# zyhbili/Dual-Space-NeRF

Measured on AMD Instinct MI355X. Metric: rendered rays/sec (64 samples/ray), 512x512 frame, higher is better.
Workload: dtype split-f16x3 (3 x v_mfma_f32_32x32x16_f16 on hi/lo fp16 operand halves, f32 accumulate: f32-equivalent accuracy - parity bars of the tests: 1e-4 absolute on RGB / acc / weights against the reference; sigma 1e-4 absolute where |sigma| <= 100 and 4e-6 RELATIVE to max|sigma| above (this checkpoint: |sig

## Files before the change

dual-space-nerf_amd/csrc/dsn_field16.hip:

```cpp
#include "dsn_common.h"
#include "dsn_kernels.h"

typedef float f32x16 __attribute__((ext_vector_type(16)));
typedef _Float16 half8 __attribute__((ext_vector_type(8)));
#define MFMA16(a, b, c) __builtin_amdgcn_mfma_f32_32x32x16_f16((a), (b), (c), 0, 0, 0)

#if !defined(DSN_EXPERIMENTS) && (defined(F16_ABL) || defined(F16_SABL) || defined(F16_TIMING) || defined(F16_TRAIN_ABL))
#error "F16_ABL / F16_SABL / F16_TIMING are experiment switches (wrong results / debug counters): build with -DDSN_EXPERIMENTS"
#endif
#ifndef F16_SINCOS_OCML
#define F16_SINCOS_OCML 0
#endif
#ifndef F16_FENCE
#define F16_FENCE 0
#endif
#ifndef F16_SGB
#define F16_SGB 1
#endif
#ifndef F16_SGB_VALU
#define F16_SGB_VALU 2
#endif
#ifndef F16_SGB_DS
#define F16_SGB_DS 1
#endif
#ifndef F16_MIX
#define F16_MIX 1
#endif
#ifndef F16_PIPE_LATE
#define F16_PIPE_LATE 1
#endif
#ifndef F16_ABL
#define F16_ABL 0
#endif
#ifndef F16_NEXT_POINT
#define F16_NEXT_POINT 1
#endif
#ifndef F16_DMA_SPREAD
#define F16_DMA_SPREAD 1
#endif
#ifndef F16_BIAS_AHEAD
#define F16_BIAS_AHEAD 1
#endif
#ifndef F16_TIMING
#define F16_TIMING 0
#endif
#ifndef F16_PREFETCH
#define F16_PREFETCH 1
#endif

#define F16_THREADS 256
#if defined(DSN_EXPERIMENTS) && defined(F16_TRAIN_ABL) && (F16_TRAIN_ABL & 32)
#define F16_ST_M(m) (1024 * (m))
#else
#define F16_ST_M(m) (32 * (m))
#endif
#define F16_CHUNK 8
#define F16_RING_SLOTS (2 * F16_CHUNK)
#define F16_NCHUNK (DSN_STREAM_BLOCKS / F16_CHUNK)
#define F16_RANGE 65000.0f
#define F16_RANGE_SCALED 32768.0f
#define F16_GSCALE 0.015625f
#define F16_GUNSCALE 64.0f

#if F16_TIMING
__device__ unsigned long long g_f16_timing[16];
#define F16_STAMP(i) do { if (MODE == F16_FWD) { asm volatile("s_waitcnt vmcnt(0) lgkmcnt(0)" ::: "memory"); tstamp[i] = __builtin_readcyclecounter(); rstamp[i] = wall_clock64(); } } while (0)
extern "C" __attribute__((visibility("default"))) int dsn_debug_timing(unsigned long long* out16, int reset) {
    if (out16 && hipMemcpyFromSymbol(out16, HIP_SYMBOL(g_f16_timing), sizeof(unsigned long long) * 16) != hipSuccess) return 1;
    if (reset) { unsigned long long z[16] = {0}; if (hipMemcpyToSymbol(HIP_SYMBOL(g_f16_timing), z, sizeof(z)) != hipSuccess) return 1; }
    return 0;
}
#else
#define F16_STAMP(i) do { } while (0)
#endif
struct W16 {
    const char* g;
    char* ring;
    unsigned ring_off;
    int wave;
    int nchunk = F16_NCHUNK;
    bool spread = F16_DMA_SPREAD != 0;
    half8 h0, l0, h1, l1;
};

#ifndef F16_POS_OFFS
#define F16_POS_OFFS 0
#endif
__device__ __forceinline__ void w16_stage(const W16& w, int c) {
    const char* src = w.g + (size_t)c * 32768;
    const unsigned dst = w.ring_off + (c & 1) * 32768 + w.wave * 8192 + 4096;
#if F16_POS_OFFS
    asm volatile("s_mov_b32 m0, %1\n\ts_nop 0\n\t"
                 "global_load_lds_dwordx4 %0, off\n\tglobal_load_lds_dwordx4 %0, off offset:1024\n\t"
                 "global_load_lds_dwordx4 %0, off offset:2048\n\tglobal_load_lds_dwordx4 %0, off offset:3072"
                 : : "v"(src - 4096), "s"(dst - 4096) : "memory", "m0");
    asm volatile("s_mov_b32 m0, %1\n\ts_nop 0\n\t"
                 "global_load_lds_dwordx4 %0, off\n\tglobal_load_lds_dwordx4 %0, off offset:1024\n\t"
                 "global_load_lds_dwordx4 %0, off offset:2048\n\tglobal_load_lds_dwordx4 %0, off offset:3072"
                 : : "v"(src), "s"(dst) : "memory", "m0");
    return;
#endif
    asm volatile("s_mov_b32 m0, %1\n\ts_nop 0\n\t"
                 "global_load_lds_dwordx4 %0, off offset:-4096\n\tglobal_load_lds_dwordx4 %0, off offset:-3072\n\t"
                 "global_load_lds_dwordx4 %0, off offset:-2048\n\tglobal_load_lds_dwordx4 %0, off offset:-1024\n\t"
                 "global_load_lds_dwordx4 %0, off\n\tglobal_load_lds_dwordx4 %0, off offset:1024\n\t"
                 "global_load_lds_dwordx4 %0, off offset:2048\n\tglobal_load_lds_dwordx4 %0, off offset:3072"
                 : : "v"(src), "s"(dst) : "memory", "m0");
}
template <int I>
__device__ __forceinline__ void w16_stage_part(const W16& w, int c) {
    const char* src = w.g + (size_t)c * 32768;
    const unsigned dst = w.ring_off + (c & 1) * 32768 + w.wave * 8192 + 4096;
#if F16_POS_OFFS
    {
        const int back = I < 2 ? 4096 : 0;
        asm volatile("s_mov_b32 m0, %1\n\ts_nop 0\n\t"
                     "global_load_lds_dwordx4 %0, off offset:%2\n\tglobal_load_lds_dwordx4 %0, off offset:%3"
                     : : "v"(src - back), "s"(dst - back), "n"(2048 * (I & 1)), "n"(2048 * (I & 1) + 1024) : "memory", "m0");
        return;
    }
#endif
    asm volatile("s_mov_b32 m0, %1\n\ts_nop 0\n\t"
                 "global_load_lds_dwordx4 %0, off offset:%2\n\tglobal_load_lds_dwordx4 %0, off offset:%3"
                 : : "v"(src), "s"(dst), "n"(-4096 + 2048 * I), "n"(-3072 + 2048 * I) : "memory", "m0");
}
__device__ __forceinline__ void w16_boundary(const W16& w, int b) {
#if !(F16_ABL & 2)
    asm volatile("s_waitcnt vmcnt(0)" ::: "memory");
#endif
#if !(F16_ABL & 1)
    __syncthreads();
#endif
    const int c = b / F16_CHUNK;
#if !(F16_ABL & 4)
    if (!w.spread && c + 1 < w.nchunk) w16_stage(w, c + 1);
#endif
}
__device__ __forceinline__ void w16_read(const W16& w, int b, int lane, half8& h0, half8& l0, half8& h1, half8& l1) {
    const char* s = w.ring + ((b >> 3) & 1) * 32768 + (b & 7) * 1024 + lane * 16;
    h0 = *reinterpret_cast<const half8*>(s);
    l0 = *reinterpret_cast<const half8*>(s + 8192);
    h1 = *reinterpret_cast<const half8*>(s + 16384);
    l1 = *reinterpret_cast<const half8*>(s + 24576);
}
__device__ __forceinline__ void w16_begin_issue(W16& w, int first_blk) { w16_stage(w, first_blk / F16_CHUNK); }
__device__ __forceinline__ void w16_begin_wait(W16& w, int lane, int first_blk) {
    w16_boundary(w, first_blk);
#if !(F16_ABL & 4)
    if (w.spread && first_blk / F16_CHUNK + 1 < w.nchunk) w16_stage_part<0>(w, first_blk / F16_CHUNK + 1);
#endif
    w16_read(w, first_blk, lane, w.h0, w.l0, w.h1, w.l1);
}
__device__ __forceinline__ void w16_begin(W16& w, int lane, int first_blk) {
    w16_begin_issue(w, first_blk);
    w16_begin_wait(w, lane, first_blk);
}

struct NoHook { __device__ __forceinline__ void operator()(int) const {} };

template <int KB, bool XLS, class Hook = NoHook>
__device__ __forceinline__ void dense16(W16& w, int& blk, int lane, const half8 (&xh)[KB][2], const half8 (&xl)[KB][2],
                                        f32x16& accM, f32x16& accC, Hook&& hook = NoHook()) {
#pragma unroll
    for (int kb = 0; kb < KB; ++kb) {
#if F16_PREFETCH
        half8 n0 = w.h0, m0 = w.l0, n1 = w.h1, m1 = w.l1;
        if (blk + 1 < DSN_STREAM_BLOCKS) {
            if (((blk + 1) & (F16_CHUNK - 1)) == 0) w16_boundary(w, blk + 1);
#if !(F16_ABL & 4)
            if (w.spread) {
                const int pos = (blk + 1) & (F16_CHUNK - 1), cn = (blk + 1) / F16_CHUNK + 1;
                if (cn < w.nchunk) {
                    if (pos == 0) w16_stage_part<0>(w, cn);
                    if (pos == 1) w16_stage_part<1>(w, cn);
                    if (pos == 2) w16_stage_part<2>(w, cn);
                    if (pos == 3) w16_stage_part<3>(w, cn);
                }
            }
#endif
            w16_read(w, blk + 1, lane, n0, m0, n1, m1);
        }
#else
        if (blk > 0) {
            if ((blk & (F16_CHUNK - 1)) == 0) w16_boundary(w, blk);
            w16_read(w, blk, lane, w.h0, w.l0, w.h1, w.l1);
        }
#endif
        if (XLS) {
            accM = MFMA16(w.h0, xh[kb][0], accM);
            accC = MFMA16(w.h0, xl[kb][0], accC);
            accC = MFMA16(w.l0, xh[kb][0], accC);
            accM = MFMA16(w.h1, xh[kb][1], accM);
            accC = MFMA16(w.h1, xl[kb][1], accC);
            accC = MFMA16(w.l1, xh[kb][1], accC);
        } else {
            accM = MFMA16(w.h0, xh[kb][0], accM);
            accC = MFMA16(w.l0, xh[kb][0], accC);
            accM = MFMA16(w.h0, xl[kb][0], accM);
            accC = MFMA16(w.h1, xh[kb][1], accC);
            accM = MFMA16(w.l1, xh[kb][1], accM);
            accC = MFMA16(w.h1, xl[kb][1], accC);
        }
#if !(F16_ABL & 8)
        hook(kb);
#endif
#if F16_PREFETCH
        w.h0 = n0; w.l0 = m0; w.h1 = n1; w.l1 = m1;
#endif
        ++blk;
#if F16_SGB
#pragma unroll
        for (int i = 0; i < 6; ++i) {
            __builtin_amdgcn_sched_group_barrier(0x008, 1, 0);
#if F16_SGB_DS
            if (i < 4) __builtin_amdgcn_sched_group_barrier(0x100, 1, 0);
#endif
            __builtin_amdgcn_sched_group_barrier(0x002, F16_SGB_VALU, 0);
        }
        __builtin_amdgcn_sched_barrier(0);
#endif
#if F16_FENCE
        __builtin_amdgcn_sched_barrier(0);
#endif
    }
}

__device__ __forceinline__ f32x16 rows16(const float* __restrict__ v, int m, int half) {
    f32x16 o;
#pragma unroll
    for (int q = 0; q < 4; ++q) {
        const float4 t = *reinterpret_cast<const float4*>(v + 32 * m + 8 * q + 4 * half);
        o[4 * q + 0] = t.x; o[4 * q + 1] = t.y; o[4 * q + 2] = t.z; o[4 * q + 3] = t.w;
    }
    return o;
}
__device__ __forceinline__ f32x16 zero16() {
    f32x16 z;
#pragma unroll
    for (int r = 0; r < 16; ++r) z[r] = 0.0f;
    return z;
}
template <bool SCALED>
__device__ __forceinline__ void split16(const f32x16& v, half8 (&h)[2], half8 (&l)[2]) {
#pragma unroll
    for (int r = 0; r < 16; ++r) {
        const _Float16 hi = (_Float16)v[r];
        const float res = fmaf((float)hi, -1.0f, v[r]);
        h[r >> 3][r & 7] = hi;
        l[r >> 3][r & 7] = SCALED ? (_Float16)(res * DSN_LO_SCALE) : (_Float16)res;
    }
}
#define F16_FWD_SCALE 64.0f
#define F16_FWD_INV 0.015625f
__device__ __forceinline__ f32x16 unscale16(const f32x16& m, const f32x16& c) {
    f32x16 v;
#pragma unroll
    for (int r = 0; r < 16; ++r) v[r] = (m[r] + c[r]) * F16_FWD_INV;
    return v;
}
__device__ __forceinline__ f32x16 fold16(const f32x16& m, const f32x16& c) {
    f32x16 v;
#pragma unroll
    for (int r = 0; r < 16; ++r) v[r] = fmaf(c[r], DSN_LO_INV, m[r]);
    return v;
}
__device__ __forceinline__ uint32_t dsn_push_sign(uint32_t word, float v) {
    return __builtin_amdgcn_alignbit(word, __float_as_uint(v), 31);
}
__device__ __forceinline__ uint32_t dsn_active_word(uint32_t signs) { return ~signs & 0xffffu; }
#ifndef F16_KEEP_ASM
#define F16_KEEP_ASM 1
#endif
__device__ __forceinline__ float dsn_keep_active(float v, uint32_t word, int r) {
#if F16_KEEP_ASM
    uint32_t m;
    asm("v_bfe_i32 %0, %1, %2, 1" : "=v"(m) : "v"(word), "s"(15 - r));
    return __uint_as_float(__float_as_uint(v) & m);
#else
    return __uint_as_float(__float_as_uint(v) & (uint32_t)__builtin_amdgcn_sbfe((int)word, 15 - r, 1));
#endif
}
__device__ __forceinline__ uint32_t relu_bits16(f32x16& a) {
    uint32_t s = 0;
#pragma unroll
    for (int r = 0; r < 16; ++r) {
        s = dsn_push_sign(s, a[r]);
        a[r] = fmaxf(a[r], 0.0f);
    }
    return dsn_active_word(s);
}
__device__ __forceinline__ void mask16(f32x16& a, uint32_t m) {
#pragma unroll
    for (int r = 0; r < 16; ++r) a[r] = dsn_keep_active(a[r], m, r);
}

__device__ __forceinline__ void track16(float& ovf, const f32x16& v) {
#pragma unroll
    for (int r = 0; r < 16; r += 2) asm("v_max3_f32 %0, %0, |%1|, |%2|" : "+v"(ovf) : "v"(v[r]), "v"(v[r + 1]));
}
__device__ __forceinline__ float dsn_nan_flag() { return __uint_as_float(0x7fc00000u); }

#if defined(DSN_EXPERIMENTS) && defined(F16_TRAIN_ABL) && (F16_TRAIN_ABL & 256)
__device__ __forceinline__ void store16_lines_emul(float* st, const float (&o)[16]) {
    const int lane = threadIdx.x & 63;
    const unsigned long long me = (unsigned long long)(uintptr_t)st;
#pragma unroll
    for (int j = 0; j < 4; ++j) {
        const int src = 8 * j + (lane >> 3);
        const unsigned lo = __shfl((unsigned)me, src), hi = __shfl((unsigned)(me >> 32), src);
        float* pj = reinterpret_cast<float*>((uintptr_t)(((unsigned long long)hi << 32) | lo));
        if (pj) *reinterpret_cast<float4*>(pj + 4 * (lane & 7)) = make_float4(o[4 * j], o[4 * j + 1], o[4 * j + 2], o[4 * j + 3]);
    }
}
#endif
template <bool FWD, bool ST = false, bool HEAD = false>
__device__ __forceinline__ void epi_slice(const f32x16& pM, const f32x16& pC, int kb, uint32_t mword, uint32_t& bits,
                                          half8 (&yh)[2], half8 (&yl)[2], float& ovf, float* st = nullptr, float stscale = 1.0f,
                                          const float* wd = nullptr, float* sg = nullptr) {
#if F16_ABL & 16
    {
        asm volatile("" : : "a"(pM[2 * kb]), "a"(pM[2 * kb + 1]), "a"(pC[2 * kb]), "a"(pC[2 * kb + 1]));
        if (kb == 0) { yh[0] = yh[1]; yl[0] = yl[1]; }
        return;
    }
#endif
    float vv[2];
#pragma unroll
    for (int e = 0; e < 2; ++e) {
        const int r = 2 * kb + e;
// ... 71 lines not shown
    }
}
#ifndef F16_NT_STORE
#define F16_NT_STORE 0
#endif
typedef float f32x4 __attribute__((ext_vector_type(4)));
__device__ __forceinline__ void store16(float* st, const f32x16& v, float stscale) {
#if defined(DSN_EXPERIMENTS) && defined(F16_TRAIN_ABL) && (F16_TRAIN_ABL & 4)
    {
        const int lane = threadIdx.x & 63, hf = lane >> 5, i = lane & 3;
        const unsigned long long me = (unsigned long long)(uintptr_t)st;
#pragma unroll
        for (int j = 0; j < 4; ++j) {
            const int src = (lane & ~3) | j;
            const unsigned lo = __shfl((unsigned)me, src), hi = __shfl((unsigned)(me >> 32), src);
            float* pj = reinterpret_cast<float*>((uintptr_t)(((unsigned long long)hi << 32) | lo));
            if (pj) *reinterpret_cast<float4*>(pj - 4 * hf + 16 * hf + 4 * i) =
                make_float4(v[4 * j] * stscale, v[4 * j + 1] * stscale, v[4 * j + 2] * stscale, v[4 * j + 3] * stscale);
        }
        return;
    }
#endif
#if defined(DSN_EXPERIMENTS) && defined(F16_TRAIN_ABL) && (F16_TRAIN_ABL & 256)
    {
        float o[16];
#pragma unroll
        for (int r = 0; r < 16; ++r) o[r] = v[r] * stscale;
        store16_lines_emul(st, o);
        return;
    }
#endif
    if (!st) return;
#pragma unroll
    for (int q = 0; q < 4; ++q) {
#if F16_NT_STORE
        const f32x4 x = {v[4 * q] * stscale, v[4 * q + 1] * stscale, v[4 * q + 2] * stscale, v[4 * q + 3] * stscale};
        __builtin_nontemporal_store(x, reinterpret_cast<f32x4*>(st + 8 * q));
#else
        *reinterpret_cast<float4*>(st + 8 * q) = make_float4(v[4 * q] * stscale, v[4 * q + 1] * stscale, v[4 * q + 2] * stscale, v[4 * q + 3] * stscale);
#endif
    }
}

template <bool ST = false, bool EXTRA = false, bool HEAD = false>
__device__ __forceinline__ void layer16_fwd(W16& w, int& blk, int lane, const float* __restrict__ bias,
                                            const half8 (&xh)[8][2], const half8 (&xl)[8][2], half8 (&yh)[8][2],
                                            half8 (&yl)[8][2], uint32_t (&mk)[4], float& ovf, float* st = nullptr,
                                            const half8 (*s_pe)[F16_THREADS] = nullptr, const float* wden = nullptr, float* sg = nullptr) {
    const int half = lane >> 5;
    const int tid = threadIdx.x;
    f32x16 pM = zero16(), pC = zero16();
#if F16_BIAS_AHEAD
    f32x16 bnext = rows16(bias, 0, half);
#endif
#pragma unroll
    for (int m = 0; m < 8; ++m) {
#if F16_BIAS_AHEAD
        f32x16 aM = bnext, aC = zero16();
        if (m + 1 < 8) bnext = rows16(bias, m + 1, half);
#else
        f32x16 aM = rows16(bias, m, half), aC = zero16();
#endif
        uint32_t bits = 0;
        if (m == 0) dense16<8, false>(w, blk, lane, xh, xl, aM, aC);
        else dense16<8, false>(w, blk, lane, xh, xl, aM, aC, [&](int kb) {
            epi_slice<true, ST, HEAD>(pM, pC, kb, 0u, bits, yh[m - 1], yl[m - 1], ovf, (ST && st) ? st + F16_ST_M(m - 1) : nullptr, 1.0f,
                                      HEAD ? wden + 32 * (m - 1) + 4 * half : nullptr, sg); });
        if (EXTRA) {
            half8 qh[2][2], ql[2][2];
            qh[0][0] = s_pe[0][tid]; qh[0][1] = s_pe[1][tid]; qh[1][0] = s_pe[2][tid]; qh[1][1] = s_pe[3][tid];
            ql[0][0] = s_pe[4][tid]; ql[0][1] = s_pe[5][tid]; ql[1][0] = s_pe[6][tid]; ql[1][1] = s_pe[7][tid];
            dense16<2, false>(w, blk, lane, qh, ql, aM, aC);
        }
        if (m > 0) { if ((m - 1) & 1) mk[(m - 1) >> 1] |= dsn_active_word(bits) << 16; else mk[(m - 1) >> 1] = dsn_active_word(bits); }
        pM = aM; pC = aC;
    }
    {
        uint32_t bits = 0;
#pragma unroll
        for (int kb = 0; kb < 8; ++kb)
            epi_slice<true, ST, HEAD>(pM, pC, kb, 0u, bits, yh[7], yl[7], ovf, (ST && st) ? st + F16_ST_M(7) : nullptr, 1.0f,
                                      HEAD ? wden + 32 * 7 + 4 * half : nullptr, sg);
        mk[3] |= dsn_active_word(bits) << 16;
    }
}
template <bool ST = false>
__device__ __forceinline__ void layer16_bwd(W16& w, int& blk, int lane, const half8 (&xh)[8][2],
                                            const half8 (&xl)[8][2], half8 (&yh)[8][2], half8 (&yl)[8][2],
                                            const uint32_t (&mk)[4], float& ovf, float* st = nullptr, float stscale = F16_GUNSCALE) {
    f32x16 pM = zero16(), pC = zero16();
    uint32_t dummy = 0;
#pragma unroll
    for (int m = 0; m < 8; ++m) {
        f32x16 aM = zero16(), aC = zero16();
        const uint32_t mw = m > 0 ? ((mk[(m - 1) >> 1] >> (16 * ((m - 1) & 1))) & 0xffffu) : 0u;
        if (m == 0) dense16<8, true>(w, blk, lane, xh, xl, aM, aC);
        else dense16<8, true>(w, blk, lane, xh, xl, aM, aC, [&](int kb) { epi_slice<false, ST>(pM, pC, kb, mw, dummy, yh[m - 1], yl[m - 1], ovf, (ST && st) ? st + F16_ST_M(m - 1) : nullptr, stscale); });
        pM = aM; pC = aC;
    }
    const uint32_t mw = (mk[3] >> 16) & 0xffffu;
#pragma unroll
    for (int kb = 0; kb < 8; ++kb) epi_slice<false, ST>(pM, pC, kb, mw, dummy, yh[7], yl[7], ovf, (ST && st) ? st + F16_ST_M(7) : nullptr, stscale);
}

#define F16_FULL 0
#define F16_FWD 1
#define F16_BWD 2
#define F16_TRAIN 3
#define F16_DEN 4
#define F16_FIRST_BWD_BLOCK (OFF_L6T / DSN_BLK)
#define F16_DEN_BLOCKS (F16_FIRST_BWD_BLOCK - 4 * 8)
static_assert(F16_DEN_BLOCKS % F16_CHUNK == 0, "the density-only kernel streams whole chunks");
template <int MODE>
__global__ void __launch_bounds__(F16_THREADS, 1)
k_field16(const float* __restrict__ packed, const DsnFrameState* __restrict__ fs, const float* __restrict__ x_c,
          int64_t N, const int32_t* __restrict__ active_list, const int32_t* __restrict__ active_count,
          float* __restrict__ sigma, float* __restrict__ essence, float* __restrict__ grad,
          uint4* __restrict__ masks, int32_t* __restrict__ pos_list, int32_t* __restrict__ pos_count,
          float* __restrict__ tr_h, float* __restrict__ tr_a, float* __restrict__ tr_rr, int64_t slot_base, int64_t rec_cap,
          const int32_t* __restrict__ sel, int32_t* __restrict__ flag_count) {
    constexpr bool ST = MODE == F16_TRAIN;
    __shared__ __attribute__((aligned(16))) char ring[F16_RING_SLOTS * 4096];
    __shared__ uint32_t s_mask[7][4][F16_THREADS];
    __shared__ __attribute__((aligned(16))) float s_vec[256 + 2304 + 8];
    __shared__ __attribute__((aligned(16))) half8 s_pe[8][F16_THREADS];
    __shared__ int s_app[8];
#ifndef F16_SHARE_SIMD
    DSN_OWN_SIMD();
#endif
    const int tid0 = threadIdx.x;
    const int lane0 = threadIdx.x & 63;
    const int wave = __builtin_amdgcn_readfirstlane(threadIdx.x >> 6);
    int64_t count = (active_list ? (int64_t)(*active_count) : N) - slot_base;
    if (MODE == F16_BWD && count > rec_cap) count = rec_cap;
    const int64_t ntiles = (count + 127) / 128;
    if ((int64_t)blockIdx.x >= ntiles) return;
    for (int i = tid0; i < 256 + 2304 + 8; i += F16_THREADS)
        s_vec[i] = i < 256 ? fs->bias0[i] : (i < 2560 ? packed[OFF_B1 + (i - 256)] : packed[OFF_SCAL + (i - 2560)]);
    for (int i = tid0; i < 256 + (OFF_WDEN - OFF_B1); i += F16_THREADS) s_vec[i] *= F16_FWD_SCALE;
    const float* const v_bias0 = s_vec;
    const float* const v_b1 = s_vec + 256;
    const float* const v_brgb1 = s_vec + 256 + (OFF_BRGB1 - OFF_B1);
    const float* const v_wden = s_vec + 256 + (OFF_WDEN - OFF_B1);
    const float* const v_wrgb3 = s_vec + 256 + (OFF_WRGB3 - OFF_B1);
    const float* const v_scal = s_vec + 2560;
    W16 w;
    w.g = reinterpret_cast<const char*>(packed + OFF16_BASE) + wave * 8192 + 4096 + lane0 * 16;
    w.ring = ring;
    w.ring_off = (unsigned)(uintptr_t)(__attribute__((address_space(3))) char*)ring;
    w.wave = wave;
    if (MODE == F16_FWD) w.nchunk = F16_FIRST_BWD_BLOCK / F16_CHUNK;
    if (MODE == F16_DEN) w.nchunk = F16_DEN_BLOCKS / F16_CHUNK;
    if (MODE == F16_TRAIN) w.spread = false;
    auto tile_point = [&](int64_t t, bool& ok, int64_t& ls) -> int64_t {
        int64_t sl = (t * 4 + wave) * 32 + (lane0 & 31);
        ok = sl < count;
        if (!ok) sl = count - 1;
        ls = sel ? (int64_t)sel[sl] : slot_base + sl;
        return active_list ? (int64_t)active_list[ls] : ls;
    };
    bool valid_n;
    int64_t lslot_n;
    int64_t pt_n = tile_point(blockIdx.x, valid_n, lslot_n);
    float xn[3] = {x_c[3 * pt_n], x_c[3 * pt_n + 1], x_c[3 * pt_n + 2]};
  for (int64_t tile = blockIdx.x; tile < ntiles; tile += gridDim.x) {
    int tid = tid0, lane = lane0;
    asm volatile("" : "+v"(tid), "+v"(lane), "+v"(w.g));
    const int half = lane >> 5;
#if F16_TIMING
    unsigned long long tstamp[6], rstamp[6];
#endif
    F16_STAMP(0);
    w16_begin_issue(w, MODE == F16_BWD ? F16_FIRST_BWD_BLOCK : 0);
#if !F16_NEXT_POINT
    if (tile != (int64_t)blockIdx.x) { pt_n = tile_point(tile, valid_n, lslot_n); xn[0] = x_c[3 * pt_n]; xn[1] = x_c[3 * pt_n + 1]; xn[2] = x_c[3 * pt_n + 2]; }
#endif
    const bool valid = valid_n;
    const int64_t lslot = lslot_n, pt = pt_n;
    const float xa[3] = {xn[0], xn[1], xn[2]};
    const bool more = F16_NEXT_POINT && MODE != F16_TRAIN && tile + gridDim.x < ntiles;
    if (more) pt_n = tile_point(tile + gridDim.x, valid_n, lslot_n);
#define NEXT_POINT() do { if (more) { xn[0] = x_c[3 * pt_n]; xn[1] = x_c[3 * pt_n + 1]; xn[2] = x_c[3 * pt_n + 2]; } } while (0)
    w16_begin_wait(w, lane, MODE == F16_BWD ? F16_FIRST_BWD_BLOCK : 0);
    int blk = MODE == F16_BWD ? F16_FIRST_BWD_BLOCK : 0;
    F16_STAMP(1);

#define MK_STORE(L, mk) { if (MODE != F16_DEN) { s_mask[L][0][tid] = mk[0]; s_mask[L][1][tid] = mk[1]; s_mask[L][2][tid] = mk[2]; s_mask[L][3][tid] = mk[3]; } }
#define MK_LOAD(L, mk) { mk[0] = s_mask[L][0][tid]; mk[1] = s_mask[L][1][tid]; mk[2] = s_mask[L][2][tid]; mk[3] = s_mask[L][3][tid]; }
    uint32_t mk[4];
    half8 ah[8][2], al[8][2], bh[8][2], bl[8][2];
    float ovf = packed[DSN_SPLIT_UNSAFE_FIELD];
    uint4* mrec = masks ? masks + ((size_t)(MODE == F16_BWD ? lslot : pt) * 2 + half) * 7 : nullptr;
    const int64_t tr_ls = N * 256;
#if defined(DSN_EXPERIMENTS) && defined(F16_TRAIN_ABL)
    const int64_t pt_st = (F16_TRAIN_ABL & 8) ? (pt & 4095) : ((F16_TRAIN_ABL & 16) ? (pt & 255) : pt);
    const int64_t sl_st = (tile * 4 + wave) * 32 + (lane & 31);
    const int64_t row_off = (F16_TRAIN_ABL & 32) ? (sl_st >> 5) * 8192 + (sl_st & 31) * 32 : pt_st * 256;
    float* const th = ST && valid && !(F16_TRAIN_ABL & 1) ? tr_h + row_off + 4 * half : nullptr;
    float* const ta = ST && valid && !(F16_TRAIN_ABL & 2) ? tr_a + row_off + 4 * half : nullptr;
#else
    float* const th = ST && valid ? tr_h + pt * 256 + 4 * half : nullptr;
    float* const ta = ST && valid ? tr_a + pt * 256 + 4 * half : nullptr;
#endif

  if (MODE != F16_BWD) {
    half8 ph[2][2], pl[2][2];
    {
        f32x16 pe[2];
#pragma unroll
        for (int t = 0; t < 30; ++t) {
            float s, c;
#if F16_SINCOS_OCML
            sincosf(xa[t % 3] * (float)(1 << (t / 3)), &s, &c);
#else
            dsn_sincos(xa[t % 3] * (float)(1 << (t / 3)), s, c);
#endif
            pe[t >> 4][t & 15] = half ? c : s;
        }
        pe[1][14] = half ? xa[1] : xa[0];
        pe[1][15] = half ? 0.0f : xa[2];
        split16<false>(pe[0], ph[0], pl[0]);
        split16<false>(pe[1], ph[1], pl[1]);
        s_pe[0][tid] = ph[0][0]; s_pe[1][tid] = ph[0][1]; s_pe[2][tid] = ph[1][0]; s_pe[3][tid] = ph[1][1];
        s_pe[4][tid] = pl[0][0]; s_pe[5][tid] = pl[0][1]; s_pe[6][tid] = pl[1][0]; s_pe[7][tid] = pl[1][1];
    }

    F16_STAMP(2);
#pragma unroll
    for (int m = 0; m < 8; ++m) {
        f32x16 aM = rows16(v_bias0, m, half), aC = zero16();
        dense16<2, false>(w, blk, lane, ph, pl, aM, aC);
        f32x16 v = unscale16(aM, aC);
        const uint32_t bits = relu_bits16(v);
        if (m & 1) mk[m >> 1] |= bits << 16; else mk[m >> 1] = bits;
        if (ST) store16(th ? th + 0 * tr_ls + F16_ST_M(m) : nullptr, v, 1.0f);
        track16(ovf, v);
        split16<false>(v, ah[m], al[m]);
    }
    MK_STORE(0, mk)
    layer16_fwd<ST>(w, blk, lane, v_b1 + 0 * 256, ah, al, bh, bl, mk, ovf, th ? th + 1 * tr_ls : nullptr); MK_STORE(1, mk)
    NEXT_POINT();
    layer16_fwd<ST>(w, blk, lane, v_b1 + 1 * 256, bh, bl, ah, al, mk, ovf, th ? th + 2 * tr_ls : nullptr); MK_STORE(2, mk)
    layer16_fwd<ST>(w, blk, lane, v_b1 + 2 * 256, ah, al, bh, bl, mk, ovf, th ? th + 3 * tr_ls : nullptr); MK_STORE(3, mk)
#if F16_PIPE_LATE
    layer16_fwd<ST, true, false>(w, blk, lane, v_b1 + 3 * 256, bh, bl, ah, al, mk, ovf, th ? th + 4 * tr_ls : nullptr, s_pe);
    MK_STORE(4, mk)
    layer16_fwd<ST>(w, blk, lane, v_b1 + 4 * 256, ah, al, bh, bl, mk, ovf, th ? th + 5 * tr_ls : nullptr); MK_STORE(5, mk)
    float sg_part = 0.0f;
    layer16_fwd<ST, false, true>(w, blk, lane, v_b1 + 5 * 256, bh, bl, ah, al, mk, ovf, th ? th + 6 * tr_ls : nullptr, nullptr, v_wden,
                                 &sg_part);
#else
#pragma unroll
    for (int m = 0; m < 8; ++m) {
        f32x16 aM = rows16(v_b1 + 3 * 256, m, half), aC = zero16();
        dense16<8, false>(w, blk, lane, bh, bl, aM, aC);
        {
            half8 qh[2][2], ql[2][2];
            qh[0][0] = s_pe[0][tid]; qh[0][1] = s_pe[1][tid]; qh[1][0] = s_pe[2][tid]; qh[1][1] = s_pe[3][tid];
            ql[0][0] = s_pe[4][tid]; ql[0][1] = s_pe[5][tid]; ql[1][0] = s_pe[6][tid]; ql[1][1] = s_pe[7][tid];
            dense16<2, false>(w, blk, lane, qh, ql, aM, aC);
        }
        f32x16 v = unscale16(aM, aC);
        const uint32_t bits = relu_bits16(v);
        if (m & 1) mk[m >> 1] |= bits << 16; else mk[m >> 1] = bits;
        if (ST) store16(th ? th + 4 * tr_ls + F16_ST_M(m) : nullptr, v, 1.0f);
        track16(ovf, v);
        split16<false>(v, ah[m], al[m]);
    }
    MK_STORE(4, mk)
    layer16_fwd<ST>(w, blk, lane, v_b1 + 4 * 256, ah, al, bh, bl, mk, ovf, th ? th + 5 * tr_ls : nullptr); MK_STORE(5, mk)
    float sg_part = 0.0f;
#pragma unroll
    for (int m = 0; m < 8; ++m) {
        f32x16 aM = rows16(v_b1 + 5 * 256, m, half), aC = zero16();
        dense16<8, false>(w, blk, lane, bh, bl, aM, aC);
        f32x16 v = unscale16(aM, aC);
        const uint32_t bits = relu_bits16(v);
        if (m & 1) mk[m >> 1] |= bits << 16; else mk[m >> 1] = bits;
        if (ST) store16(th ? th + 6 * tr_ls + F16_ST_M(m) : nullptr, v, 1.0f);
        const f32x16 wd = rows16(v_wden, m, half);
#pragma unroll
        for (int r = 0; r < 16; ++r) sg_part = fmaf(wd[r], v[r], sg_part);
        track16(ovf, v);
        split16<false>(v, ah[m], al[m]);
    }
#endif
    F16_STAMP(3);
    sg_part += __shfl_xor(sg_part, 32);
    const float sg = sg_part + v_scal[0];
    const bool flag_fwd = !(fmaxf(ovf, __shfl_xor(ovf, 32)) < F16_RANGE);
    if (valid && half == 0) sigma[pt] = flag_fwd ? dsn_nan_flag() : sg;
    if (MODE != F16_TRAIN && flag_fwd && valid && half == 0 && flag_count) atomicAdd(flag_count, 1);
    ovf = flag_fwd ? __builtin_inff() : 0.0f;
    if (MODE == F16_DEN) { __syncthreads(); continue; }
    bool write_rec = ST && valid;
    if (MODE == F16_FWD) {
        const bool pos = valid && half == 0 && (sg > 0.0f || flag_fwd);
        const unsigned long long bm = __ballot(pos);
        const int cnt = __popcll(bm);
        if (lane == 0) s_app[wave] = cnt;
        __syncthreads();
        if (tid == 0) {
            const int tot = s_app[0] + s_app[1] + s_app[2] + s_app[3];
            s_app[4] = tot ? atomicAdd(pos_count, tot) : 0;
        }
        __syncthreads();
        int base = s_app[4];
        for (int k = 0; k < wave; ++k) base += s_app[k];
        const int my = base + __popcll(bm & ((1ull << lane) - 1ull));
        if (pos) pos_list[my] = (int32_t)pt;
        const int rslot = __shfl(my, lane & 31);
        write_rec = ((bm >> (lane & 31)) & 1ull) != 0 && (int64_t)rslot < rec_cap;
        mrec = masks + ((size_t)rslot * 2 + half) * 7;
    }
    if (MODE == F16_FWD || MODE == F16_TRAIN) {
        MK_STORE(6, mk)
        if (write_rec) {
#pragma unroll
            for (int L = 0; L < 7; ++L)
                mrec[L] = make_uint4(s_mask[L][0][tid], s_mask[L][1][tid], s_mask[L][2][tid], s_mask[L][3][tid]);
        }
    }
    {
        float e0 = 0.f, e1 = 0.f, e2 = 0.f;
#pragma unroll
        for (int m = 0; m < 4; ++m) {
            f32x16 aM = rows16(v_brgb1, m, half), aC = zero16();
            dense16<8, false>(w, blk, lane, ah, al, aM, aC);
            const f32x16 v = unscale16(aM, aC);
            const f32x16 w0 = rows16(v_wrgb3 + 0 * 128, m, half);
            const f32x16 w1 = rows16(v_wrgb3 + 1 * 128, m, half);
            const f32x16 w2 = rows16(v_wrgb3 + 2 * 128, m, half);
            if (ST && valid) {
                f32x16 xr;
#pragma unroll
                for (int r = 0; r < 16; ++r) xr[r] = fmaxf(v[r], 0.0f);
                store16(tr_rr + pt * 128 + 4 * half + 32 * m, xr, 1.0f);
            }
#pragma unroll
            for (int r = 0; r < 16; ++r) {
                const float x = fmaxf(v[r], 0.0f);
                e0 = fmaf(w0[r], x, e0); e1 = fmaf(w1[r], x, e1); e2 = fmaf(w2[r], x, e2);
            }
        }
        e0 += __shfl_xor(e0, 32); e1 += __shfl_xor(e1, 32); e2 += __shfl_xor(e2, 32);
        if (valid && half == 0) {
            essence[3 * pt + 0] = e0 + v_scal[1];
            essence[3 * pt + 1] = e1 + v_scal[2];
            essence[3 * pt + 2] = e2 + v_scal[3];
        }
    }

#if F16_TIMING
    F16_STAMP(4);
    if (MODE == F16_FWD && tid == 0) {
        for (int i = 0; i < 4; ++i) { atomicAdd(&g_f16_timing[i], tstamp[i + 1] - tstamp[i]); atomicAdd(&g_f16_timing[8 + i], rstamp[i + 1] - rstamp[i]); }
        atomicAdd(&g_f16_timing[7], 1ull);
    }
#endif
    if (MODE == F16_FWD) { __syncthreads(); continue; }
  } else {
#pragma unroll
    for (int L = 0; L < 7; ++L) {
        const uint4 q = mrec[L];
        s_mask[L][0][tid] = q.x; s_mask[L][1][tid] = q.y; s_mask[L][2][tid] = q.z; s_mask[L][3][tid] = q.w;
    }
    MK_LOAD(6, mk)
  }

#pragma unroll
    for (int m = 0; m < 8; ++m) {
        f32x16 g = rows16(v_wden, m, half);
#pragma unroll
        for (int r = 0; r < 16; ++r) g[r] *= F16_GSCALE;
        mask16(g, (mk[m >> 1] >> (16 * (m & 1))) & 0xffffu);
        if (ST) store16(ta ? ta + 6 * tr_ls + F16_ST_M(m) : nullptr, g, F16_GUNSCALE);
        split16<true>(g, ah[m], al[m]);
    }
    MK_LOAD(5, mk) layer16_bwd<ST>(w, blk, lane, ah, al, bh, bl, mk, ovf, ta ? ta + 5 * tr_ls : nullptr);
    if (MODE == F16_BWD) NEXT_POINT();
    MK_LOAD(4, mk) layer16_bwd<ST>(w, blk, lane, bh, bl, ah, al, mk, ovf, ta ? ta + 4 * tr_ls : nullptr);
    MK_LOAD(3, mk)
    f32x16 dpe[2];
#pragma unroll
    for (int m = 0; m < 8; ++m) {
        f32x16 aM = zero16(), aC = zero16();
        dense16<8, true>(w, blk, lane, ah, al, aM, aC);
        f32x16 v = fold16(aM, aC);
        mask16(v, (mk[m >> 1] >> (16 * (m & 1))) & 0xffffu);
        if (ST) store16(ta ? ta + 3 * tr_ls + F16_ST_M(m) : nullptr, v, F16_GUNSCALE);
        track16(ovf, v);
        split16<true>(v, bh[m], bl[m]);
    }
#pragma unroll
    for (int b = 0; b < 2; ++b) {
        f32x16 aM = zero16(), aC = zero16();
        dense16<8, true>(w, blk, lane, ah, al, aM, aC);
        dpe[b] = fold16(aM, aC);
    }
    MK_LOAD(2, mk) layer16_bwd<ST>(w, blk, lane, bh, bl, ah, al, mk, ovf, ta ? ta + 2 * tr_ls : nullptr);
    MK_LOAD(1, mk) layer16_bwd<ST>(w, blk, lane, ah, al, bh, bl, mk, ovf, ta ? ta + 1 * tr_ls : nullptr);
    MK_LOAD(0, mk) layer16_bwd<ST>(w, blk, lane, bh, bl, ah, al, mk, ovf, ta ? ta + 0 * tr_ls : nullptr);
#pragma unroll
    for (int b = 0; b < 2; ++b) {
        f32x16 aM = zero16(), aC = zero16();
        dense16<8, true>(w, blk, lane, ah, al, aM, aC);
        const f32x16 v = fold16(aM, aC);
#pragma unroll
        for (int r = 0; r < 16; ++r) dpe[b][r] += v[r];
    }

    {
        float xb[3] = {xa[0], xa[1], xa[2]};
        asm volatile("" : "+v"(xb[0]), "+v"(xb[1]), "+v"(xb[2]));
        float g[3] = {0.f, 0.f, 0.f};
#pragma unroll
        for (int t = 0; t < 30; ++t) {
            const int j = t / 3, a = t % 3;
            float s, c;
#if F16_SINCOS_OCML
            sincosf(xb[a] * (float)(1 << j), &s, &c);
#else
            dsn_sincos(xb[a] * (float)(1 << j), s, c);
#endif
            const float d = dpe[t >> 4][t & 15];
            const float term = (d * (half ? s : c)) * (float)(1 << j);
            g[a] += half ? -term : term;
        }
        const float i30 = dpe[1][14], i31 = dpe[1][15];
        if (half) g[1] += i30; else { g[0] += i30; g[2] += i31; }
        g[0] += __shfl_xor(g[0], 32); g[1] += __shfl_xor(g[1], 32); g[2] += __shfl_xor(g[2], 32);
        if (valid && half == 0) {
            grad[3 * pt] = g[0] * F16_GUNSCALE; grad[3 * pt + 1] = g[1] * F16_GUNSCALE; grad[3 * pt + 2] = g[2] * F16_GUNSCALE;
        }
    }
    const bool flagged = !(fmaxf(ovf, __shfl_xor(ovf, 32)) < F16_RANGE_SCALED);
    if (flagged && valid && half == 0) {
        if (MODE == F16_TRAIN) { if (pos_count) atomicAdd(pos_count, 1); }
        else { sigma[pt] = dsn_nan_flag(); if (flag_count) atomicAdd(flag_count, 1); }
    }
    if (MODE == F16_TRAIN) break;
    __syncthreads();
  }
}

void dsn_launch_field16(const float* packed, const DsnFrameState* fs, const float* x_c, int64_t N,
                        const int32_t* active_list, const int32_t* active_count, float* sigma, float* essence,
                        float* grad, hipStream_t st, int32_t* flag_count) {
    int64_t blocks = (N + 127) / 128;
    if (blocks == 0) return;
    hipLaunchKernelGGL(k_field16<F16_FULL>, dim3((unsigned)std::min<int64_t>(blocks, dsn_cu_count())), dim3(F16_THREADS), 0, st, packed, fs, x_c, N,
                       active_list, active_count, sigma, essence, grad, (uint4*)nullptr, (int32_t*)nullptr,
                       (int32_t*)nullptr, (float*)nullptr, (float*)nullptr, (float*)nullptr, (int64_t)0, (int64_t)0, (const int32_t*)nullptr,
                       flag_count);
}
void dsn_launch_field16_from(const float* packed, const DsnFrameState* fs, const float* x_c, int64_t N, const int32_t* list,
                             const int32_t* count, int64_t slot_base, float* sigma, float* essence, float* grad, hipStream_t st,
                             int32_t* flag_count) {
    int64_t blocks = (N - slot_base + 127) / 128;
    if (blocks <= 0) return;
    hipLaunchKernelGGL(k_field16<F16_FULL>, dim3((unsigned)std::min<int64_t>(blocks, dsn_cu_count())), dim3(F16_THREADS), 0, st, packed, fs, x_c, N, list, count, sigma,
                       essence, grad, (uint4*)nullptr, (int32_t*)nullptr, (int32_t*)nullptr, (float*)nullptr, (float*)nullptr,
                       (float*)nullptr, slot_base, (int64_t)0, (const int32_t*)nullptr, flag_count);
}
void dsn_launch_field16_train(const float* packed, const DsnFrameState* fs, const float* x_c, int64_t N, float* sigma,
                              float* essence, float* grad, float* tr_h, float* tr_a, float* tr_rr, void* masks, hipStream_t st,
                              int32_t* range_count, const int32_t* row_list, const int32_t* row_count) {
    int64_t blocks = (N + 127) / 128;
    if (blocks == 0) return;
    hipLaunchKernelGGL(k_field16<F16_TRAIN>, dim3((unsigned)blocks), dim3(F16_THREADS), 0, st, packed, fs, x_c, N,
                       row_list, row_count, sigma, essence, grad, (uint4*)masks, (int32_t*)nullptr,
                       range_count, tr_h, tr_a, tr_rr, (int64_t)0, N, (const int32_t*)nullptr, (int32_t*)nullptr);
}
void dsn_launch_field16_fwd(const float* packed, const DsnFrameState* fs, const float* x_c, int64_t N,
                            const int32_t* active_list, const int32_t* active_count, float* sigma, float* essence,
                            void* masks, int32_t* pos_list, int32_t* pos_count, hipStream_t st, int64_t rec_cap, int32_t* flag_count) {
    int64_t blocks = (N + 127) / 128;
    if (blocks == 0) return;
    hipLaunchKernelGGL(k_field16<F16_FWD>, dim3((unsigned)std::min<int64_t>(blocks, dsn_cu_count())), dim3(F16_THREADS), 0, st, packed, fs, x_c, N,
                       active_list, active_count, sigma, essence, (float*)nullptr, (uint4*)masks, pos_list, pos_count,
                       (float*)nullptr, (float*)nullptr, (float*)nullptr, (int64_t)0, rec_cap, (const int32_t*)nullptr, flag_count);
}
void dsn_launch_field16_den(const float* packed, const DsnFrameState* fs, const float* x_c, int64_t N,
                            const int32_t* active_list, const int32_t* active_count, float* sigma, hipStream_t st,
                            int32_t* flag_count) {
    int64_t blocks = (N + 127) / 128;
    if (blocks == 0) return;
    hipLaunchKernelGGL(k_field16<F16_DEN>, dim3((unsigned)std::min<int64_t>(blocks, dsn_cu_count())), dim3(F16_THREADS), 0, st, packed, fs, x_c, N,
                       active_list, active_count, sigma, (float*)nullptr, (float*)nullptr, (uint4*)nullptr, (int32_t*)nullptr,
                       (int32_t*)nullptr, (float*)nullptr, (float*)nullptr, (float*)nullptr, (int64_t)0, (int64_t)0,
                       (const int32_t*)nullptr, flag_count);
}
void dsn_launch_field16_bwd(const float* packed, const DsnFrameState* fs, const float* x_c, int64_t N,
                            const int32_t* pos_list, const int32_t* pos_count, float* grad, const void* masks,
                            hipStream_t st, float* sigma, int64_t rec_cap, const int32_t* sel, const int32_t* sel_count,
                            int32_t* flag_count) {
    int64_t blocks = ((rec_cap < N ? rec_cap : N) + 127) / 128;
    if (blocks == 0) return;
    hipLaunchKernelGGL(k_field16<F16_BWD>, dim3((unsigned)std::min<int64_t>(blocks, dsn_cu_count())), dim3(F16_THREADS), 0, st, packed, fs, x_c, N,
                       pos_list, sel ? sel_count : pos_count, sigma, (float*)nullptr, grad, (uint4*)masks, (int32_t*)nullptr,
                       (int32_t*)nullptr, (float*)nullptr, (float*)nullptr, (float*)nullptr, (int64_t)0, rec_cap, sel, flag_count);
}

__device__ __forceinline__ void epi_slice_tan(const f32x16& pM, const f32x16& pC, int kb, uint32_t mword, half8 (&yh)[2],
                                              half8 (&yl)[2], float* st, float stscale, float& ovf, float* keep = nullptr) {
    float vv[2];
#pragma unroll
    for (int e = 0; e < 2; ++e) {
        const int r = 2 * kb + e;
        const float v = dsn_keep_active((pM[r] + pC[r]) * F16_FWD_INV, mword, r);
        vv[e] = v;
        const _Float16 hi = (_Float16)v;
        yh[r >> 3][r & 7] = hi;
        yl[r >> 3][r & 7] = (_Float16)fmaf((float)hi, -1.0f, v);
    }
    asm("v_max3_f32 %0, %0, |%1|, |%2|" : "+v"(ovf) : "v"(vv[0]), "v"(vv[1]));
#if defined(DSN_EXPERIMENTS) && defined(F16_TRAIN_ABL) && (F16_TRAIN_ABL & 256)
    if (kb == 7) {
        float o[16];
#pragma unroll
        for (int r = 0; r < 16; ++r) o[r] = dsn_keep_active((pM[r] + pC[r]) * F16_FWD_INV, mword, r) * stscale;
        store16_lines_emul(st, o);
        return;
    }
#endif
    if (keep && kb == 7) {
#pragma unroll
        for (int r = 0; r < 16; ++r) keep[r] = dsn_keep_active((pM[r] + pC[r]) * F16_FWD_INV, mword, r) * stscale;
        return;
    }
    if (st && kb == 7) {
#pragma unroll
        for (int q = 0; q < 4; ++q) {
            float o[4];
#pragma unroll
            for (int e = 0; e < 4; ++e) o[e] = dsn_keep_active((pM[4 * q + e] + pC[4 * q + e]) * F16_FWD_INV, mword, 4 * q + e) * stscale;
            *reinterpret_cast<float4*>(st + 8 * q) = make_float4(o[0], o[1], o[2], o[3]);
        }
    }
}
__device__ __forceinline__ void layer16_tan(W16& w, int& blk, int lane, const half8 (&xh)[8][2], const half8 (&xl)[8][2],
                                            half8 (&yh)[8][2], half8 (&yl)[8][2], const uint32_t (&mk)[4], float* st, float stscale,
                                            float& ovf, float (*keep)[16] = nullptr) {
    f32x16 pM = zero16(), pC = zero16();
#pragma unroll
    for (int m = 0; m < 8; ++m) {
        f32x16 aM = zero16(), aC = zero16();
        const uint32_t mw = m > 0 ? ((mk[(m - 1) >> 1] >> (16 * ((m - 1) & 1))) & 0xffffu) : 0u;
        if (m == 0) dense16<8, false>(w, blk, lane, xh, xl, aM, aC);
        else dense16<8, false>(w, blk, lane, xh, xl, aM, aC, [&](int kb) { epi_slice_tan(pM, pC, kb, mw, yh[m - 1], yl[m - 1], st ? st + 32 * (m - 1) : nullptr, stscale, ovf, keep ? keep[m - 1] : nullptr); });
        pM = aM; pC = aC;
    }
    const uint32_t mw = (mk[3] >> 16) & 0xffffu;
#pragma unroll
    for (int kb = 0; kb < 8; ++kb) epi_slice_tan(pM, pC, kb, mw, yh[7], yl[7], st ? st + 32 * 7 : nullptr, stscale, ovf, keep ? keep[7] : nullptr);
}

__device__ __forceinline__ float half_wave_sum_to_last(float v) {
    v += __builtin_bit_cast(float, __builtin_amdgcn_update_dpp(0, __builtin_bit_cast(int, v), 0x111, 0xf, 0xf, true));
    v += __builtin_bit_cast(float, __builtin_amdgcn_update_dpp(0, __builtin_bit_cast(int, v), 0x112, 0xf, 0xf, true));
    v += __builtin_bit_cast(float, __builtin_amdgcn_update_dpp(0, __builtin_bit_cast(int, v), 0x114, 0xf, 0xf, true));
    v += __builtin_bit_cast(float, __builtin_amdgcn_update_dpp(0, __builtin_bit_cast(int, v), 0x118, 0xf, 0xf, true));
    v += __builtin_bit_cast(float, __builtin_amdgcn_update_dpp(0, __builtin_bit_cast(int, v), 0x142, 0xa, 0xf, true));
    return v;
}

__device__ __forceinline__ void zero_train_rows(float* t, int64_t ls, int layers) {
    for (int L = 0; L < layers; ++L)
        for (int m = 0; m < 8; ++m)
#pragma unroll
            for (int q = 0; q < 4; ++q) *reinterpret_cast<float4*>(t + L * ls + 32 * m + 8 * q) = make_float4(0.f, 0.f, 0.f, 0.f);
}

__global__ void __launch_bounds__(F16_THREADS, 1)
k_tangent16(const float* __restrict__ packed, const float* __restrict__ x_c, const float* __restrict__ u, int64_t N,
            const uint4* __restrict__ masks, float* __restrict__ tr_t, uint32_t* __restrict__ gmax, int32_t* __restrict__ range_count,
            const int32_t* __restrict__ row_list, const int32_t* __restrict__ row_count, float* __restrict__ colsum6) {
    __shared__ __attribute__((aligned(16))) char ring[F16_RING_SLOTS * 4096];
    __shared__ uint32_t s_mask[7][4][F16_THREADS];
    __shared__ __attribute__((aligned(16))) half8 s_pe[8][F16_THREADS];
    DSN_OWN_SIMD_T(1);
    const int tid = threadIdx.x;
    const int lane = threadIdx.x & 63;
    const int wave = __builtin_amdgcn_readfirstlane(threadIdx.x >> 6);
    const int half = lane >> 5;
    const int64_t NL = row_count ? (int64_t)(*row_count) : N;
    if ((int64_t)blockIdx.x * 128 >= NL) return;
    int64_t pt = ((int64_t)blockIdx.x * 4 + wave) * 32 + (lane & 31);
    const bool valid = pt < NL;
    if (!valid) pt = NL - 1;
    if (row_list) pt = (int64_t)row_list[pt];
    const float xa[3] = {x_c[3 * pt], x_c[3 * pt + 1], x_c[3 * pt + 2]};
    float ua[3] = {u[3 * pt], u[3 * pt + 1], u[3 * pt + 2]};
    float sc = fmaxf(fmaxf(fabsf(ua[0]), fabsf(ua[1])), fabsf(ua[2]));
    if (!(sc > 1e-30f) || !(sc < 3.0e38f)) sc = 0.0f;
    const float inv = sc > 0.0f ? 0.015625f / sc : 0.0f;
// ... 1223 lines not shown
```

Baseline: 29.39 million.

## Carry tile outputs and wrap weight prefetch into next tile in persistent field kernel

In the forward and density modes of the persistent field kernel, the weight-stream prefetch now wraps so the next tile's first chunk is staged during the current tile's last chunk. Each tile's sigma, essence, flag and mask-record writes are deferred and flushed at the start of the next tile, with a final flush after the loop. The per-tile __syncthreads pair for the compacted-append atomic is also removed by hiding the atomic inside the RGB head's MFMA loop. This is meant to remove the pipeline drain and barrier stalls at tile boundaries. The cost is more live registers for the carried state and more complex ring-buffer ordering, including a required even chunk count.

```diff
diff --git a/dual-space-nerf_amd/csrc/dsn_field16.hip b/dual-space-nerf_amd/csrc/dsn_field16.hip
--- a/dual-space-nerf_amd/csrc/dsn_field16.hip
+++ b/dual-space-nerf_amd/csrc/dsn_field16.hip
@@ -80,6 +80,7 @@
     int wave;
     int nchunk = F16_NCHUNK;
     bool spread = F16_DMA_SPREAD != 0;
+    bool wrap = false;
     half8 h0, l0, h1, l1;
 };
 
@@ -165,7 +166,7 @@
     for (int kb = 0; kb < KB; ++kb) {
 #if F16_PREFETCH
         half8 n0 = w.h0, m0 = w.l0, n1 = w.h1, m1 = w.l1;
-        if (blk + 1 < DSN_STREAM_BLOCKS) {
+        if (blk + 1 < w.nchunk * F16_CHUNK) {
             if (((blk + 1) & (F16_CHUNK - 1)) == 0) w16_boundary(w, blk + 1);
 #if !(F16_ABL & 4)
             if (w.spread) {
@@ -175,6 +176,11 @@
                     if (pos == 1) w16_stage_part<1>(w, cn);
                     if (pos == 2) w16_stage_part<2>(w, cn);
                     if (pos == 3) w16_stage_part<3>(w, cn);
+                } else if (cn == w.nchunk && w.wrap) {
+                    if (pos == 0) w16_stage_part<0>(w, 0);
+                    if (pos == 1) w16_stage_part<1>(w, 0);
+                    if (pos == 2) w16_stage_part<2>(w, 0);
+                    if (pos == 3) w16_stage_part<3>(w, 0);
                 }
             }
 #endif
@@ -552,6 +558,29 @@
     if (MODE == F16_FWD) w.nchunk = F16_FIRST_BWD_BLOCK / F16_CHUNK;
     if (MODE == F16_DEN) w.nchunk = F16_DEN_BLOCKS / F16_CHUNK;
     if (MODE == F16_TRAIN) w.spread = false;
+    constexpr bool CARRY = MODE == F16_FWD || MODE == F16_DEN;
+    static_assert(!CARRY || ((MODE == F16_FWD ? F16_FIRST_BWD_BLOCK : F16_DEN_BLOCKS) / F16_CHUNK) % 2 == 0,
+                  "the wrapped fetch needs an even chunk count: the last chunk in ring half 1, the next tile's first in half 0");
+    int64_t c_pt = 0;
+    float c_sig = 0.0f, c_e0 = 0.0f, c_e1 = 0.0f, c_e2 = 0.0f;
+    int c_slot = 0;
+    unsigned c_do = 0;
+    auto flush_tile = [&](int tid, int half) {
+        if (c_do & 1u) {
+            sigma[c_pt] = c_sig;
+            if (MODE == F16_FWD) { essence[3 * c_pt + 0] = c_e0; essence[3 * c_pt + 1] = c_e1; essence[3 * c_pt + 2] = c_e2; }
+        }
+        if ((c_do & 2u) && flag_count) atomicAdd(flag_count, 1);
+        if (MODE == F16_FWD) {
+            if (c_do & 4u) pos_list[c_slot] = (int32_t)c_pt;
+            if (c_do & 8u) {
+                uint4* const rec = masks + ((size_t)c_slot * 2 + half) * 7;
+#pragma unroll
+                for (int L = 0; L < 7; ++L)
+                    rec[L] = make_uint4(s_mask[L][0][tid], s_mask[L][1][tid], s_mask[L][2][tid], s_mask[L][3][tid]);
+            }
+        }
+    };
     auto tile_point = [&](int64_t t, bool& ok, int64_t& ls) -> int64_t {
         int64_t sl = (t * 4 + wave) * 32 + (lane0 & 31);
         ok = sl < count;
@@ -563,15 +592,16 @@
     int64_t lslot_n;
     int64_t pt_n = tile_point(blockIdx.x, valid_n, lslot_n);
     float xn[3] = {x_c[3 * pt_n], x_c[3 * pt_n + 1], x_c[3 * pt_n + 2]};
+    if (CARRY) w16_begin_issue(w, 0);
   for (int64_t tile = blockIdx.x; tile < ntiles; tile += gridDim.x) {
     int tid = tid0, lane = lane0;
     asm volatile("" : "+v"(tid), "+v"(lane), "+v"(w.g));
     const int half = lane >> 5;
 #if F16_TIMING
-    unsigned long long tstamp[6], rstamp[6];
+    unsigned long long tstamp[8], rstamp[8];
 #endif
     F16_STAMP(0);
-    w16_begin_issue(w, MODE == F16_BWD ? F16_FIRST_BWD_BLOCK : 0);
+    if (!CARRY) w16_begin_issue(w, MODE == F16_BWD ? F16_FIRST_BWD_BLOCK : 0);
 #if !F16_NEXT_POINT
     if (tile != (int64_t)blockIdx.x) { pt_n = tile_point(tile, valid_n, lslot_n); xn[0] = x_c[3 * pt_n]; xn[1] = x_c[3 * pt_n + 1]; xn[2] = x_c[3 * pt_n + 2]; }
 #endif
@@ -579,11 +609,16 @@
     const int64_t lslot = lslot_n, pt = pt_n;
     const float xa[3] = {xn[0], xn[1], xn[2]};
     const bool more = F16_NEXT_POINT && MODE != F16_TRAIN && tile + gridDim.x < ntiles;
-    if (more) pt_n = tile_point(tile + gridDim.x, valid_n, lslot_n);
+    if (!CARRY && more) pt_n = tile_point(tile + gridDim.x, valid_n, lslot_n);
 #define NEXT_POINT() do { if (more) { xn[0] = x_c[3 * pt_n]; xn[1] = x_c[3 * pt_n + 1]; xn[2] = x_c[3 * pt_n + 2]; } } while (0)
+    w.wrap = CARRY && more;
     w16_begin_wait(w, lane, MODE == F16_BWD ? F16_FIRST_BWD_BLOCK : 0);
     int blk = MODE == F16_BWD ? F16_FIRST_BWD_BLOCK : 0;
     F16_STAMP(1);
+    if (CARRY) {
+        if (more) pt_n = tile_point(tile + gridDim.x, valid_n, lslot_n);
+        flush_tile(tid, half);
+    }
 
 #define MK_STORE(L, mk) { if (MODE != F16_DEN) { s_mask[L][0][tid] = mk[0]; s_mask[L][1][tid] = mk[1]; s_mask[L][2][tid] = mk[2]; s_mask[L][3][tid] = mk[3]; } }
 #define MK_LOAD(L, mk) { mk[0] = s_mask[L][0][tid]; mk[1] = s_mask[L][1][tid]; mk[2] = s_mask[L][2][tid]; mk[3] = s_mask[L][3][tid]; }
@@ -639,13 +674,14 @@
     }
     MK_STORE(0, mk)
     layer16_fwd<ST>(w, blk, lane, v_b1 + 0 * 256, ah, al, bh, bl, mk, ovf, th ? th + 1 * tr_ls : nullptr); MK_STORE(1, mk)
-    NEXT_POINT();
+    if (!CARRY) NEXT_POINT();
     layer16_fwd<ST>(w, blk, lane, v_b1 + 1 * 256, bh, bl, ah, al, mk, ovf, th ? th + 2 * tr_ls : nullptr); MK_STORE(2, mk)
     layer16_fwd<ST>(w, blk, lane, v_b1 + 2 * 256, ah, al, bh, bl, mk, ovf, th ? th + 3 * tr_ls : nullptr); MK_STORE(3, mk)
 #if F16_PIPE_LATE
     layer16_fwd<ST, true, false>(w, blk, lane, v_b1 + 3 * 256, bh, bl, ah, al, mk, ovf, th ? th + 4 * tr_ls : nullptr, s_pe);
     MK_STORE(4, mk)
     layer16_fwd<ST>(w, blk, lane, v_b1 + 4 * 256, ah, al, bh, bl, mk, ovf, th ? th + 5 * tr_ls : nullptr); MK_STORE(5, mk)
+    if (CARRY) NEXT_POINT();
     float sg_part = 0.0f;
     layer16_fwd<ST, false, true>(w, blk, lane, v_b1 + 5 * 256, bh, bl, ah, al, mk, ovf, th ? th + 6 * tr_ls : nullptr, nullptr, v_wden,
                                  &sg_part);
@@ -689,30 +725,27 @@
     sg_part += __shfl_xor(sg_part, 32);
     const float sg = sg_part + v_scal[0];
     const bool flag_fwd = !(fmaxf(ovf, __shfl_xor(ovf, 32)) < F16_RANGE);
-    if (valid && half == 0) sigma[pt] = flag_fwd ? dsn_nan_flag() : sg;
-    if (MODE != F16_TRAIN && flag_fwd && valid && half == 0 && flag_count) atomicAdd(flag_count, 1);
+    if (CARRY) {
+        c_pt = pt;
+        c_sig = flag_fwd ? dsn_nan_flag() : sg;
+        c_do = valid && half == 0 ? (flag_fwd ? 3u : 1u) : 0u;
+    } else {
+        if (valid && half == 0) sigma[pt] = flag_fwd ? dsn_nan_flag() : sg;
+        if (MODE != F16_TRAIN && flag_fwd && valid && half == 0 && flag_count) atomicAdd(flag_count, 1);
+    }
     ovf = flag_fwd ? __builtin_inff() : 0.0f;
-    if (MODE == F16_DEN) { __syncthreads(); continue; }
-    bool write_rec = ST && valid;
+    F16_STAMP(4);
+    if (MODE == F16_DEN) continue;
+    const bool write_rec = ST && valid;
+    unsigned long long bm = 0;
+    int app_base = 0;
     if (MODE == F16_FWD) {
         const bool pos = valid && half == 0 && (sg > 0.0f || flag_fwd);
-        const unsigned long long bm = __ballot(pos);
-        const int cnt = __popcll(bm);
-        if (lane == 0) s_app[wave] = cnt;
-        __syncthreads();
-        if (tid == 0) {
-            const int tot = s_app[0] + s_app[1] + s_app[2] + s_app[3];
-            s_app[4] = tot ? atomicAdd(pos_count, tot) : 0;
-        }
-        __syncthreads();
-        int base = s_app[4];
-        for (int k = 0; k < wave; ++k) base += s_app[k];
-        const int my = base + __popcll(bm & ((1ull << lane) - 1ull));
-        if (pos) pos_list[my] = (int32_t)pt;
-        const int rslot = __shfl(my, lane & 31);
-        write_rec = ((bm >> (lane & 31)) & 1ull) != 0 && (int64_t)rslot < rec_cap;
-        mrec = masks + ((size_t)rslot * 2 + half) * 7;
-    }
+        bm = __ballot(pos);
+        if (lane == 0) s_app[wave] = __popcll(bm);
+        if (pos) c_do |= 4u;
+    }
+    F16_STAMP(5);
     if (MODE == F16_FWD || MODE == F16_TRAIN) {
         MK_STORE(6, mk)
         if (write_rec) {
@@ -721,12 +754,22 @@
                 mrec[L] = make_uint4(s_mask[L][0][tid], s_mask[L][1][tid], s_mask[L][2][tid], s_mask[L][3][tid]);
         }
     }
+    F16_STAMP(6);
     {
         float e0 = 0.f, e1 = 0.f, e2 = 0.f;
 #pragma unroll
         for (int m = 0; m < 4; ++m) {
             f32x16 aM = rows16(v_brgb1, m, half), aC = zero16();
-            dense16<8, false>(w, blk, lane, ah, al, aM, aC);
+            if (MODE == F16_FWD && m == 1)
+                dense16<8, false>(w, blk, lane, ah, al, aM, aC, [&](int kb) { if (kb == 6 && tid == 0) s_app[4] = app_base; });
+            else
+                dense16<8, false>(w, blk, lane, ah, al, aM, aC);
+            if (MODE == F16_FWD && m == 0 && tid == 0) {
+                const int tot = s_app[0] + s_app[1] + s_app[2] + s_app[3];
+                uintptr_t pc = (uintptr_t)pos_count;
+                asm volatile("" : "+v"(pc));
+                app_base = tot ? __hip_atomic_fetch_add((__attribute__((address_space(1))) int32_t*)pc, tot, __ATOMIC_RELAXED, __HIP_MEMORY_SCOPE_AGENT) : 0;
+            }
             const f32x16 v = unscale16(aM, aC);
             const f32x16 w0 = rows16(v_wrgb3 + 0 * 128, m, half);
             const f32x16 w1 = rows16(v_wrgb3 + 1 * 128, m, half);
@@ -744,7 +787,14 @@
             }
         }
         e0 += __shfl_xor(e0, 32); e1 += __shfl_xor(e1, 32); e2 += __shfl_xor(e2, 32);
-        if (valid && half == 0) {
+        if (MODE == F16_FWD) {
+            c_e0 = e0 + v_scal[1]; c_e1 = e1 + v_scal[2]; c_e2 = e2 + v_scal[3];
+            int base = s_app[4];
+            for (int k = 0; k < wave; ++k) base += s_app[k];
+            const int my = base + __popcll(bm & ((1ull << lane) - 1ull));
+            c_slot = __shfl(my, lane & 31);
+            if (((bm >> (lane & 31)) & 1ull) != 0 && (int64_t)c_slot < rec_cap) c_do |= 8u;
+        } else if (valid && half == 0) {
             essence[3 * pt + 0] = e0 + v_scal[1];
             essence[3 * pt + 1] = e1 + v_scal[2];
             essence[3 * pt + 2] = e2 + v_scal[3];
@@ -752,13 +802,13 @@
     }
 
 #if F16_TIMING
-    F16_STAMP(4);
+    F16_STAMP(7);
     if (MODE == F16_FWD && tid == 0) {
-        for (int i = 0; i < 4; ++i) { atomicAdd(&g_f16_timing[i], tstamp[i + 1] - tstamp[i]); atomicAdd(&g_f16_timing[8 + i], rstamp[i + 1] - rstamp[i]); }
+        for (int i = 0; i < 7; ++i) { atomicAdd(&g_f16_timing[i], tstamp[i + 1] - tstamp[i]); atomicAdd(&g_f16_timing[8 + i], rstamp[i + 1] - rstamp[i]); }
         atomicAdd(&g_f16_timing[7], 1ull);
     }
 #endif
-    if (MODE == F16_FWD) { __syncthreads(); continue; }
+    if (MODE == F16_FWD) continue;
   } else {
 #pragma unroll
     for (int L = 0; L < 7; ++L) {
@@ -842,6 +892,7 @@
     if (MODE == F16_TRAIN) break;
     __syncthreads();
   }
+    if (CARRY) flush_tile(tid0, lane0 >> 5);
 }
 
 void dsn_launch_field16(const float* packed, const DsnFrameState* fs, const float* x_c, int64_t N,
```

After: 29.40 million (median of 4 runs). About the same (+0.0%).
